# nevi-me/rust-dataframe

Hardware: AMD Instinct MI355X
Metric: rows/sec filter+sum over 1e9 f64 Arrow rows; %HBM bw at 1/2/4/8 GPU (higher is better)
Workload: dtype f64

## Files before the change

rust_dataframe_amd/csrc/rdf_capi.cpp:

```cpp
#include <hip/hip_runtime.h>

#include <algorithm>
#include <cmath>
#include <cstdarg>
#include <cstdio>
#include <chrono>
#include <functional>
#include <cstring>
#include <map>
#include <memory>
#include <mutex>
#include <condition_variable>
#include <string>
#include <thread>
#include <vector>
#include <sys/syscall.h>
#include <unistd.h>

#include "rdf_device.h"
#include "rdf_stage_copy.h"
#include "rdf_utf8.h"
#include "rdf_colstats.h"
#include "rdf_window.h"
#include "rdf_window_agg.h"
// ... 59 lines not shown
    int    opt_gb_partition = 3;
    bool   timing = false;
    std::vector<std::pair<hipEvent_t, hipEvent_t>> events;
    size_t events_used = 0;
    std::multimap<size_t, void*> pool_free;
    size_t pool_cached = 0;
    int64_t opt_stream_slab = 0;
    void*  sbuf_dev[2] = {nullptr, nullptr};
    void*  sbuf_pin[2] = {nullptr, nullptr};
    size_t sbuf_dev_cap = 0, sbuf_pin_cap = 0;
    hipEvent_t sbuf_ev[2] = {nullptr, nullptr};
    void*  dbuf_dev[2] = {nullptr, nullptr};
    void*  dbuf_pin[2] = {nullptr, nullptr};
    size_t dbuf_dev_cap = 0, dbuf_pin_cap = 0;
    hipEvent_t dbuf_ev[2] = {nullptr, nullptr};
    hipStream_t d2h_stream = nullptr;
    int64_t stream_slabs = 0, stream_bytes_staged = 0, stream_bytes_direct = 0;
    bool in_stream = false;
    bool streaming = false;
    int  opt_stream_table_kernel = 1;
    char* tab_pin = nullptr; size_t tab_pin_cap = 0, tab_pin_used = 0;
    bool   agg_comm_entered = false;
    ::rdf_comm* agg_comm = nullptr;
    ~Ctx();
};

thread_local Ctx g_ctx;

Ctx::~Ctx() {
    if (!ready || (long)syscall(SYS_gettid) == (long)getpid()) return;
    (void)hipSetDevice(device);
    if (stream) (void)hipStreamSynchronize(stream);
    for (void* p : arena.overflow) (void)hipFree(p);
    if (arena.base) (void)hipFree(arena.base);
    if (pinned) (void)hipHostFree(pinned);
    for (auto& kv : pool_free) (void)hipFree(kv.second);
    for (int b = 0; b < 2; ++b) { if (sbuf_dev[b]) (void)hipFree(sbuf_dev[b]); if (sbuf_pin[b]) (void)hipHostFree(sbuf_pin[b]); if (sbuf_ev[b]) (void)hipEventDestroy(sbuf_ev[b]); }
    if (tab_pin) (void)hipHostFree(tab_pin);
    if (d2h_stream) (void)hipStreamSynchronize(d2h_stream);
    for (int b = 0; b < 2; ++b) { if (dbuf_dev[b]) (void)hipFree(dbuf_dev[b]); if (dbuf_pin[b]) (void)hipHostFree(dbuf_pin[b]); if (dbuf_ev[b]) (void)hipEventDestroy(dbuf_ev[b]); }
    if (d2h_stream) (void)hipStreamDestroy(d2h_stream);
    for (auto& ev : events) { (void)hipEventDestroy(ev.first); (void)hipEventDestroy(ev.second); }
    if (copy_stream) { (void)hipStreamSynchronize(copy_stream); (void)hipStreamDestroy(copy_stream); }
    if (own_stream) (void)hipStreamDestroy(own_stream);
    ready = false;
}

rdf_status fail(rdf_status st, const char* fmt, ...) {
    char buf[512];
    va_list ap;
    va_start(ap, fmt);
    vsnprintf(buf, sizeof buf, fmt, ap);
    va_end(ap);
    g_ctx.err = buf;
    if (g_ctx.ready && g_ctx.stream) (void)hipStreamSynchronize(g_ctx.stream);
    return st;
}

// ... 8 lines not shown
        if (_s != RDF_OK) return _s;   \
    } while (0)

rdf_status ensure_ready() {
    Ctx& c = g_ctx;
    if (c.ready) return RDF_OK;
    int n = 0;
    hipError_t e = hipGetDeviceCount(&n);
    if (e != hipSuccess || n <= 0)
        return fail(RDF_DEVICE_ERROR, "no HIP device visible (%s); librdf_mi355x has no CPU fallback",
                    e != hipSuccess ? hipGetErrorString(e) : "device count 0");
    HIP_TRY(hipGetDevice(&c.device));
    hipDeviceProp_t prop;
    HIP_TRY(hipGetDeviceProperties(&prop, c.device));
    if (strncmp(prop.gcnArchName, "gfx950", 6) != 0)
        return fail(RDF_DEVICE_ERROR, "device %d is %s; this library carries gfx950 (MI355X) code only", c.device, prop.gcnArchName);
    HIP_TRY(hipStreamCreateWithFlags(&c.own_stream, hipStreamNonBlocking));
    c.stream = c.own_stream;
    if (const char* e = getenv("RDF_SPEC_BLOCKS_PER_CU")) { const int v = atoi(e); if (v >= 0 && v <= 8) c.opt_spec_blocks = v; }
    if (const char* e = getenv("RDF_SPEC_TILE_ROT")) c.opt_spec_tile_rot = atoi(e);
    if (const char* e = getenv("RDF_SPEC_XCD_SWZ")) c.opt_spec_xcd_swz = atoi(e);
    if (const char* e = getenv("RDF_SPEC_GRID_ADJ")) c.opt_spec_grid_adj = atoi(e);
    if (const char* e = getenv("RDF_STREAM_TABLE_KERNEL")) c.opt_stream_table_kernel = atoi(e) != 0;
    if (const char* e = getenv("RDF_GSPEC_BLOCKS_PER_CU")) { const int v = atoi(e); if (v >= 0 && v <= 8) c.opt_gspec_blocks = v; }
    c.ready = true;
    return RDF_OK;
}

void arena_begin() {
    Arena& a = g_ctx.arena;
    for (void* p : a.overflow) (void)hipFree(p);
    a.overflow.clear();
    if (a.wanted > a.cap) {
        if (a.base) (void)hipFree(a.base);
        a.base = nullptr;
        a.cap = 0;
        size_t want = a.wanted + a.wanted / 4 + (1u << 20);
        void* p = nullptr;
        if (hipMalloc(&p, want) == hipSuccess) { a.base = (char*)p; a.cap = want; }
    }
    a.used = 0;
    a.wanted = 0;
}
rdf_status arena_alloc(size_t bytes, void** out) {
    Arena& a = g_ctx.arena;
    bytes = (bytes + 16 + 255) & ~(size_t)255;
// ... 3 lines not shown
        a.used += bytes;
        return RDF_OK;
    }
    void* p = nullptr;
    hipError_t e = hipMalloc(&p, bytes);
    if (e != hipSuccess) return fail(RDF_MEMORY_ERROR, "hipMalloc(%zu) failed: %s", bytes, hipGetErrorString(e));
    a.overflow.push_back(p);
    *out = p;
    return RDF_OK;
}
rdf_status pinned_reserve(size_t bytes) {
    Ctx& c = g_ctx;
    if (bytes <= c.pinned_cap) return RDF_OK;
    if (c.pinned && c.stream) (void)hipStreamSynchronize(c.stream);
    if (c.pinned) (void)hipHostFree(c.pinned);
    c.pinned = nullptr;
    c.pinned_cap = 0;
    size_t want = bytes + bytes / 2 + 4096;
    void* p = nullptr;
    hipError_t e = hipHostMalloc(&p, want, hipHostMallocDefault);
    if (e != hipSuccess) return fail(RDF_MEMORY_ERROR, "hipHostMalloc(%zu) failed: %s", want, hipGetErrorString(e));
    c.pinned = (char*)p;
    c.pinned_cap = want;
    return RDF_OK;
}

constexpr size_t kPoolGranule = (size_t)2 << 20;
constexpr size_t kPoolMaxCached = (size_t)96 << 30;
rdf_status pool_alloc(size_t bytes, void** out, size_t* got) {
    Ctx& c = g_ctx;
    const size_t gran = bytes < ((size_t)1 << 20) ? (size_t)4096 : kPoolGranule;
    const size_t want = (bytes + 256 + gran - 1) / gran * gran;
    auto it = c.pool_free.lower_bound(want);
    if (it != c.pool_free.end() && it->first <= want + want / 4 + gran) {
        *out = it->second; *got = it->first;
        c.pool_cached -= it->first;
        c.pool_free.erase(it);
        return RDF_OK;
    }
    void* p = nullptr;
    hipError_t e = hipMalloc(&p, want);
    if (e != hipSuccess && !c.pool_free.empty()) {
        if (c.stream) (void)hipStreamSynchronize(c.stream);
        for (auto& kv : c.pool_free) (void)hipFree(kv.second);
        c.pool_free.clear();
        c.pool_cached = 0;
// ... 732 lines not shown
                    h = (sw ? mir : fwd)[op - RDF_OP_GT];
                } else if (op == RDF_OP_AND) h = LH_AND;
                else if (op == RDF_OP_OR) h = LH_OR;
                else if (in.dtype == RDF_F64) {
                    if (op == RDF_OP_ADD) h = LH_F_ADD;
                    else if (op == RDF_OP_MUL) h = LH_F_MUL;
                    else if (op == RDF_OP_SUB) h = sw ? LH_F_RSUB : LH_F_SUB;
                    else if (op == RDF_OP_DIV) h = sw ? LH_F_RDIV : LH_F_DIV;
                } else if (in.dtype == RDF_I64 || in.dtype == RDF_U64) {
                    if (op == RDF_OP_ADD) h = LH_I_ADD;
                    else if (op == RDF_OP_MUL) h = LH_I_MUL;
                    else if (op == RDF_OP_SUB) h = sw ? LH_I_RSUB : LH_I_SUB;
                }
            } break;
            default: break;
        }
        if (h == LH_NONE) return false;
        lean.code[i].swapped = (uint8_t)((in.swapped & 1) | (h << 1));
    }
    return true;
}

rdf_status launch_agg_pair(const EvalArgs* ea, const FilterAggF64Args* fa, int cmp, int feat, int grid, int nvalues,
                           const int* cls, AggPartial* partials, AggPartial* result, const char* spec_sig = nullptr,
                           const SpecArgs* sa = nullptr) {
    Ctx& c = g_ctx;
    KernelTimer kt;
    if (sa) {
        const bool jit = jit_find(spec_sig) != nullptr;
        c.last_kernel = std::string("spec_kernel<") + spec_sig + ">" + (jit ? " [compiled at run time]" : "");
        const hipError_t le = launch_spec(spec_sig, *sa, grid, c.stream);
        if (le != hipSuccess && jit) { (void)hipGetLastError(); return kRetryInterpreted; }
        if (le != hipSuccess) return fail(RDF_DEVICE_ERROR, "launch_spec: %s", hipGetErrorString(le));
    }
    else if (fa) { c.last_kernel = "filter_agg_f64_kernel"; HIP_TRY(launch_filter_agg_f64(*fa, cmp, grid, c.stream)); }
    else {
        EvalArgs lean;
        if (c.opt_interp_lean && feat == 0 && lean_assign(*ea, lean)) { c.last_kernel = "eval_kernel<AGG, lean>"; HIP_TRY(launch_eval_lean(lean, SINK_AGG, grid, c.stream, c.opt_interp_lean == 2)); }
        else { c.last_kernel = "eval_kernel<AGG>"; HIP_TRY(launch_eval(*ea, SINK_AGG, feat, grid, c.stream)); }
    }
    kt.stop();
    AggFinalArgs f;
    memset(&f, 0, sizeof f);
    f.partials = partials;
    f.result = result;
    f.nblocks = grid;
    f.nvalues = nvalues;
    for (int k = 0; k < nvalues; ++k) f.value_cls[k] = cls[k];
    HIP_TRY(launch_agg_final(f, c.stream));
    return RDF_OK;
}

void fill_agg_result(rdf_agg_result* r, int dt, const AggPartial& p) {
    memset(r, 0, sizeof *r);
    r->dtype = dt;
    r->count = p.cnt;
    r->is_some = p.cnt > 0;
    if (is_float(dt)) {
        double s, a, b;
        memcpy(&s, &p.sum, 8); memcpy(&a, &p.mn, 8); memcpy(&b, &p.mx, 8);
        r->sum_f64 = dt == RDF_F32 ? (double)(float)s : s;
        if (p.cnt > 0) { r->min_f64 = a; r->max_f64 = b; }
    } else {
        r->sum_i64 = (int64_t)h_normalize_int(dt, p.sum);
// ... 601 lines not shown
                cmp = fr.op;
                if (L.kind == RDF_NODE_COLUMN && R.kind == RDF_NODE_SCALAR) { coln = &L; sc = &R; }
                else if (L.kind == RDF_NODE_SCALAR && R.kind == RDF_NODE_COLUMN) {
                    coln = &R; sc = &L;
                    cmp = fr.op == RDF_OP_GT ? RDF_OP_LT : fr.op == RDF_OP_GE ? RDF_OP_LE : fr.op == RDF_OP_LT ? RDF_OP_GT : fr.op == RDF_OP_LE ? RDF_OP_GE : fr.op;
                }
                if (coln && col_dtype[coln->column] == RDF_F64 && sc->dtype != RDF_NULLTYPE && (is_numeric(sc->dtype) || sc->dtype == RDF_BOOL)) {
                    const DevChunkCol& x = in_dev[(size_t)coln->column];
                    const DevChunkCol& y = in_dev[(size_t)vr.column];
                    const uintptr_t xa = (uintptr_t)((const double*)x.values + x.offset), ya = (uintptr_t)((const double*)y.values + y.offset);
                    if ((xa & 7) == 0 && (ya & 7) == 0 && (xa & 15) == (ya & 15)) {
                        memset(&fa, 0, sizeof fa);
                        fa.x = (const double*)x.values; fa.x_validity = x.validity; fa.x_offset = x.offset;
                        fa.y = (const double*)y.values; fa.y_validity = y.validity; fa.y_offset = y.offset;
                        fa.n = clen[0];
                        const uint64_t cu = cc.imm_for(*sc, RDF_F64);
                        memcpy(&fa.c, &cu, 8);
                        fa.partials = d_partials;
                        fast = true;
                    }
                }
            }
        }
        if (use_spec) {
            const rdf_status ls = launch_agg_pair(nullptr, nullptr, 0, 0, grid, ps.nvalues, cls, d_partials, d_result, sp.sig.c_str(), &sa);
            if (ls == kRetryInterpreted) return run_program(ps, cols, ncols, nchunks, outs, aggs, len_mismatch_msg, fc);
            RDF_TRY(ls);
        } else if (fast) {
            const int64_t per_block = (int64_t)kBlock * 4 * 2;
            int64_t want = (clen[0] + per_block - 1) / per_block;
            grid = (int)(want < (int64_t)eval_grid_limit() ? want : (int64_t)eval_grid_limit());
            if (grid < 1) grid = 1;
            d_result = d_partials + (size_t)grid * (size_t)ps.nvalues;
            RDF_TRY(launch_agg_pair(nullptr, &fa, cmp, 0, grid, 1, cls, d_partials, d_result));
        } else {
            RDF_TRY(launch_agg_pair(&ea, nullptr, 0, cc.feat(), grid, ps.nvalues, cls, d_partials, d_result));
        }
        if (ctx.agg_comm) {
            AggPartial hp[kMaxValues];
            uint32_t flags = 0;
            RDF_TRY(agg_dist_finish(*ctx.agg_comm, d_result, d_flags, ps.nvalues, cls, hp, &flags));
            if (flags & 2u) return fail(RDF_COMPUTE_ERROR, "pipeline_dist: another rank failed before the combine");
            if (flags & 1u) return fail(RDF_DIVIDE_BY_ZERO, "Divide by zero error");
            for (int v = 0; v < ps.nvalues; ++v) fill_agg_result(&aggs[v], value_dtype[v], hp[v]);
            return RDF_OK;
        }
        RDF_TRY(pinned_reserve(pin_off + 64 + sizeof(AggPartial) * kMaxValues));
        char* pin = ctx.pinned + pin_off;
        HIP_TRY(hipMemcpyAsync(pin, d_flags, 16, hipMemcpyDeviceToHost, ctx.stream));
        HIP_TRY(hipMemcpyAsync(pin + 64, d_result, sizeof(AggPartial) * (size_t)ps.nvalues, hipMemcpyDeviceToHost, ctx.stream));
        HIP_TRY(hipStreamSynchronize(ctx.stream));
        dbg.mark("kernel + result");
        uint32_t flags;
        memcpy(&flags, pin, 4);
        if (flags & 1u) return fail(RDF_DIVIDE_BY_ZERO, "Divide by zero error");
        for (int v = 0; v < ps.nvalues; ++v) {
            AggPartial p;
            memcpy(&p, pin + 64 + sizeof(AggPartial) * (size_t)v, sizeof p);
            fill_agg_result(&aggs[v], value_dtype[v], p);
        }
        return RDF_OK;
    }

    {
        KernelTimer kt;
        if (use_spec) {
            const bool jit = jit_find(sp.sig.c_str()) != nullptr;
            ctx.last_kernel = "spec_kernel<" + sp.sig + ">" + (jit ? " [compiled at run time]" : "");
            const hipError_t le = launch_spec(sp.sig.c_str(), sa, grid, ctx.stream);
            if (le != hipSuccess && jit) { (void)hipGetLastError(); return run_program(ps, cols, ncols, nchunks, outs, aggs, len_mismatch_msg, fc); }
            if (le != hipSuccess) return fail(RDF_DEVICE_ERROR, "launch_spec: %s", hipGetErrorString(le));
        }
        else {
            int64_t longest = 0;
            for (int64_t i = 0; i < nchunks; ++i) longest = std::max(longest, clen[(size_t)i]);
            EvalArgs lean;
            if (ctx.opt_interp_lean && cc.feat() == 0 && longest < ((int64_t)1 << 32) && lean_assign(ea, lean, SINK_STORE)) {
// ... 105 lines not shown
rdf_status rdf_device_count(int32_t* count) {
    if (!count) return fail(RDF_INVALID_ARGUMENT, "null pointer");
    int n = 0;
    hipError_t e = hipGetDeviceCount(&n);
    *count = e == hipSuccess ? n : 0;
    if (e != hipSuccess) return fail(RDF_DEVICE_ERROR, "hipGetDeviceCount: %s", hipGetErrorString(e));
    return RDF_OK;
}

rdf_status rdf_set_device(int32_t device) {
    Ctx& c = g_ctx;
    if (c.ready && c.device == device) return RDF_OK;
    if (c.ready) {
        (void)hipStreamSynchronize(c.stream);
        for (void* p : c.arena.overflow) (void)hipFree(p);
        c.arena.overflow.clear();
        if (c.arena.base) (void)hipFree(c.arena.base);
        c.arena = Arena();
        for (auto& ev : c.events) { (void)hipEventDestroy(ev.first); (void)hipEventDestroy(ev.second); }
        c.events.clear();
        c.events_used = 0;
        if (c.own_stream) (void)hipStreamDestroy(c.own_stream);
        c.own_stream = c.stream = nullptr;
        c.ready = false;
    }
    HIP_TRY(hipSetDevice(device));
    return ensure_ready();
}

rdf_status rdf_set_stream(void* hip_stream) {
    RDF_TRY(ensure_ready());
    g_ctx.stream = hip_stream ? (hipStream_t)hip_stream : g_ctx.own_stream;
    return RDF_OK;
}

rdf_status rdf_synchronize(void) {
    RDF_TRY(ensure_ready());
    HIP_TRY(hipStreamSynchronize(g_ctx.stream));
    return RDF_OK;
}

rdf_status rdf_dev_alloc(void** ptr, int64_t bytes) {
    if (!ptr || bytes < 0) return fail(RDF_INVALID_ARGUMENT, "bad arguments");
    RDF_TRY(ensure_ready());
    void* p = nullptr;
    hipError_t e = hipMalloc(&p, (size_t)bytes + 64);
// ... 2089 lines not shown
    RDF_TRY(ensure_ready());
    if (n > 0) HIP_TRY(launch_fill_f64(dev_ptr, n, seed, column_id, first_row, lo, hi, g_ctx.stream));
    HIP_TRY(hipStreamSynchronize(g_ctx.stream));
    return RDF_OK;
}
rdf_status rdf_fill_uniform_i64(int64_t* dev_ptr, int64_t n, uint64_t seed, uint64_t column_id, int64_t first_row, int64_t lo, int64_t hi) {
    if (hi <= lo) return fail(RDF_INVALID_ARGUMENT, "fill_uniform_i64: hi must exceed lo");
    RDF_TRY(ensure_ready());
    if (n > 0) HIP_TRY(launch_fill_i64(dev_ptr, n, seed, column_id, first_row, lo, hi, g_ctx.stream));
    HIP_TRY(hipStreamSynchronize(g_ctx.stream));
    return RDF_OK;
}
rdf_status rdf_fill_validity(uint8_t* dev_ptr, int64_t nbits, uint64_t seed, uint64_t column_id, int64_t first_row, double null_fraction) {
    RDF_TRY(ensure_ready());
    if (nbits > 0) HIP_TRY(launch_fill_validity(dev_ptr, nbits, seed, column_id, first_row, null_fraction, g_ctx.stream));
    HIP_TRY(hipStreamSynchronize(g_ctx.stream));
    return RDF_OK;
}

rdf_status rdf_set_option(const char* name, int64_t value) {
    if (!name) return fail(RDF_INVALID_ARGUMENT, "null option name");
    if (strcmp(name, "spec") == 0) g_ctx.opt_spec = value != 0;
    else if (strcmp(name, "fast_filter") == 0) g_ctx.opt_fast_filter = value != 0;
    else if (strcmp(name, "vec_bitmap") == 0) g_ctx.opt_vec_bitmap = value != 0;
    else if (strcmp(name, "gb_partition") == 0) g_ctx.opt_gb_partition = value == 2 ? 3 : (int)value;
    else if (strcmp(name, "gb_debug") == 0) g_ctx.opt_gb_debug = value == 3 ? 3 : 0;
    else if (strcmp(name, "filter_tile") == 0) g_ctx.opt_filter_tile = (int)value;
    else if (strcmp(name, "filter_one") == 0) g_ctx.opt_filter_one = value != 0;
    else if (strcmp(name, "take_rows") == 0) g_ctx.opt_take_rows = (int)value;
    else if (strcmp(name, "sort_gen") == 0 || strcmp(name, "sort_pipe") == 0 || strcmp(name, "sort_super") == 0) {}
    else if (strcmp(name, "sort_msd") == 0) g_ctx.opt_sort_msd = (int)value;
    else if (strcmp(name, "sort_sample") == 0) g_ctx.opt_sort_sample = (int)value;
    else if (strcmp(name, "stream_table_kernel") == 0) g_ctx.opt_stream_table_kernel = value != 0;
    else if (strcmp(name, "join_table") == 0) g_ctx.opt_join_table = value < 0 || value > 2 ? 2 : (int)value;
    else if (strcmp(name, "jit") == 0) g_ctx.opt_jit = (int)value;
    else if (strcmp(name, "gb_skew_plan") == 0) g_ctx.opt_gb_skew_plan = (int)value;
    else if (strcmp(name, "gb_compact") == 0) g_ctx.opt_gb_compact = (int)value;
    else if (strcmp(name, "gb_bucket") == 0) g_ctx.opt_gb_bucket = (int)value;
    else if (strcmp(name, "gb_hot") == 0) g_ctx.opt_gb_hot = (int)value;
    else if (strcmp(name, "spec_blocks_per_cu") == 0) g_ctx.opt_spec_blocks = (int)value;
    else if (strcmp(name, "spec_tile_rot") == 0) g_ctx.opt_spec_tile_rot = value < 0 ? -1 : (int)value;
    else if (strcmp(name, "spec_xcd_swz") == 0) g_ctx.opt_spec_xcd_swz = value < 0 ? -1 : value != 0;
    else if (strcmp(name, "spec_grid_adj") == 0) g_ctx.opt_spec_grid_adj = (int)value;
    else if (strcmp(name, "gspec_blocks_per_cu") == 0) g_ctx.opt_gspec_blocks = (int)value;
    else if (strcmp(name, "filter_gen") == 0) g_ctx.opt_filter_gen = (int)value;
    else if (strcmp(name, "filter_fused") == 0) g_ctx.opt_filter_fused = (int)value;
// ... 90 lines not shown
```

rust_dataframe_amd/csrc/rdf_common.hip.h:

```cpp
#pragma once
#include "rdf_device.h"

namespace rdfk {

__device__ __forceinline__ uint64_t uniform64(uint64_t v) {
    uint32_t lo = __builtin_amdgcn_readfirstlane((uint32_t)v);
    uint32_t hi = __builtin_amdgcn_readfirstlane((uint32_t)(v >> 32));
    return ((uint64_t)hi << 32) | lo;
}
__device__ __forceinline__ int wave_id() { return __builtin_amdgcn_readfirstlane((int)(threadIdx.x >> 6)); }

template <class T> using GlobalPtr = const T __attribute__((address_space(1)))*;
template <class T> using GlobalMutPtr = T __attribute__((address_space(1)))*;
template <class T> __device__ __forceinline__ GlobalPtr<T> as_global(const void* p) { return (GlobalPtr<T>)p; }
template <class T> using ConstPtr = const T __attribute__((address_space(4)))*;
template <class T> __device__ __forceinline__ ConstPtr<T> as_const(const void* p) { return (ConstPtr<T>)p; }
__device__ __forceinline__ DevChunkCol const_col(const DevChunkCol* table, int64_t i) {
    const ConstPtr<DevChunkCol> t = as_const<DevChunkCol>(table);
    DevChunkCol c;
    c.values = t[i].values; c.validity = t[i].validity; c.offset = t[i].offset;
    return c;
}
template <class T> __device__ __forceinline__ GlobalMutPtr<T> as_global_mut(void* p) { return (GlobalMutPtr<T>)p; }

// ... 109 lines not shown
    if (cls == CLS_F64) { sum = d2u(0.0); mn = mx = 0x7FF8000000000000ull; }
    else if (cls == CLS_SIGNED) { sum = 0; mn = (uint64_t)INT64_MAX; mx = (uint64_t)INT64_MIN; }
    else { sum = 0; mn = ~0ull; mx = 0; }
}
__device__ __forceinline__ void agg_merge(int cls, uint64_t& sum, uint64_t& mn, uint64_t& mx, int64_t& cnt,
                                          uint64_t s2, uint64_t mn2, uint64_t mx2, int64_t c2) {
    cnt += c2;
    if (cls == CLS_F64) {
        sum = d2u(u2d(sum) + u2d(s2));
        mn = d2u(fmin(u2d(mn), u2d(mn2)));
        mx = d2u(fmax(u2d(mx), u2d(mx2)));
    } else if (cls == CLS_SIGNED) {
        sum += s2;
        mn = (uint64_t)((int64_t)mn2 < (int64_t)mn ? (int64_t)mn2 : (int64_t)mn);
        mx = (uint64_t)((int64_t)mx2 > (int64_t)mx ? (int64_t)mx2 : (int64_t)mx);
    } else {
        sum += s2;
        mn = mn2 < mn ? mn2 : mn;
        mx = mx2 > mx ? mx2 : mx;
    }
}

__device__ __forceinline__ void block_reduce_agg(int cls, uint64_t sum, uint64_t mn, uint64_t mx, int64_t cnt,
                                                 AggPartial* lds4, AggPartial* out) {
#pragma unroll
    for (int m = 32; m >= 1; m >>= 1) {
        uint64_t s2 = shfl_xor64(sum, m), mn2 = shfl_xor64(mn, m), mx2 = shfl_xor64(mx, m);
        int64_t c2 = (int64_t)shfl_xor64((uint64_t)cnt, m);
        agg_merge(cls, sum, mn, mx, cnt, s2, mn2, mx2, c2);
    }
    const int wave = threadIdx.x >> 6;
    __syncthreads();
    if ((threadIdx.x & 63) == 0) { lds4[wave].sum = sum; lds4[wave].mn = mn; lds4[wave].mx = mx; lds4[wave].cnt = cnt; }
    __syncthreads();
    if (threadIdx.x == 0) {
        uint64_t s = lds4[0].sum, a = lds4[0].mn, b = lds4[0].mx;
        int64_t c = lds4[0].cnt;
        for (int w = 1; w < kBlock / 64; ++w) agg_merge(cls, s, a, b, c, lds4[w].sum, lds4[w].mn, lds4[w].mx, lds4[w].cnt);
        out->sum = s; out->mn = a; out->mx = b; out->cnt = c;
    }
}

__device__ __forceinline__ void trig_reduce(double x, double& r, int& q) {
    const double kd = rint(x * 6.36619772367581382433e-01);
    q = (int)kd;
    double t = fma(-kd, 1.57079632673412561417e+00, x);
    t = fma(-kd, 6.07710050630396597660e-11, t);
    t = fma(-kd, 2.02226624871116645580e-21, t);
    r = fma(-kd, 8.47842766036889956997e-32, t);
}
__device__ __forceinline__ double trig_ksin(double r) {
    const double z = r * r, v = z * r;
    const double p = fma(z, fma(z, fma(z, fma(z, 1.58969099521155010221e-10, -2.50507602534068634195e-08), 2.75573137070700676789e-06),
                                -1.98412698298579493134e-04), 8.33333333332248946124e-03);
    return fma(v, fma(z, p, -1.66666666666666324348e-01), r);
}
__device__ __forceinline__ double trig_kcos(double r) {
    const double z = r * r;
    const double p = z * fma(z, fma(z, fma(z, fma(z, fma(z, -1.13596475577881948265e-11, 2.08757232129817482790e-09), -2.75573143513906633035e-07),
                                            2.48015872894767294178e-05), -1.38888888888741095749e-03), 4.16666666666666019037e-02);
    return 1.0 - (0.5 * z - z * p);
}
// ... 214 lines not shown
```

rust_dataframe_amd/csrc/rdf_device.h:

```cpp
#pragma once
#include "rdf_sort_map.h"
#include <stdint.h>
#include <hip/hip_runtime.h>

#include <string>
#include "../../include/rdf_mi355x.h"

namespace rdfk {

constexpr int kBlock = 256;
constexpr int kVPT = 4;
constexpr int kEvalTile = kBlock * kVPT;
constexpr int kFilterTile = 4096;
constexpr int kFilterTileSmall = 1024;
constexpr int kMaxCode = 56;
constexpr int kMaxCols = 8;
constexpr int kMaxFrameCols = 64;
constexpr int kPreCols = 4;
constexpr int kMaxTmp = 4;
constexpr int kMaxValues = RDF_MAX_VALUES;
constexpr int kMaxGroupValues = RDF_MAX_GROUP_VALUES;
constexpr int kMaxFilterCols = 8;

struct DevChunkCol {
// ... 13 lines not shown
    uint8_t  bc;
    uint8_t  op;
    uint8_t  dtype;
    uint8_t  src_kind;
    uint8_t  src_dtype;
    uint8_t  swapped;
    uint16_t src;
    uint64_t imm;
};
static_assert(sizeof(Instr) == 16, "Instr must stay 16 bytes");
enum : int {
    LH_NONE = 0, LH_LOAD, LH_STORE_TMP, LH_FILTER, LH_EMIT, LH_NOT, LH_CAST_I2F, LH_CAST_U2F,
    LH_F_GT, LH_F_GE, LH_F_EQ, LH_F_NE, LH_F_LT, LH_F_LE, LH_F_ADD, LH_F_SUB, LH_F_RSUB, LH_F_MUL, LH_F_DIV, LH_F_RDIV,
    LH_I_ADD, LH_I_SUB, LH_I_RSUB, LH_I_MUL, LH_AND, LH_OR
};

struct AggPartial {
    uint64_t sum, mn, mx;
    int64_t  cnt;
};
enum : int32_t { CLS_F64 = 0, CLS_SIGNED = 1, CLS_UNSIGNED = 2 };

enum : int32_t { SINK_STORE = 0, SINK_AGG = 1, SINK_GROUP = 2 };

struct EvalArgs {
    const DevChunkCol* cols;
    const int64_t*     chunk_tile_start;
    const int64_t*     chunk_len;
    DevOutChunk*       outs;
    int64_t*           out_null_counts;
    AggPartial*        partials;
    uint64_t*          group_partials;
    uint32_t*          flags;
    int64_t            nchunks, ntiles;
    DevChunkCol        inline_cols[kMaxCols];
    DevOutChunk        inline_outs[kMaxValues];
    int64_t            inline_len;
    int32_t            ncols, nvalues, ncode, ntmp;
    int32_t            col_dtype[kMaxCols];
    int32_t            value_cls[kMaxGroupValues];
    int32_t            ngroups, group_replicas;
    Instr              code[kMaxCode];
};

inline __host__ __device__ int group_words(int ngroups, int nvalues) { return (ngroups + 1) * (2 * nvalues + 1); }

constexpr int kGSpecCols = 8;
constexpr int kGSpecImm = 8;
struct GSpecArgs {
    const DevChunkCol* cols_tab;
    const int64_t*     chunk_tile_start;
    const int64_t*     chunk_len;
    DevChunkCol        cols[kGSpecCols];
    int32_t            col_map[kGSpecCols];
    int64_t            nchunks, ntiles, n;
    uint64_t           imm[kGSpecImm];
    uint64_t*          group_partials;
    uint32_t*          flags;
    int32_t            ngroups, nvalues, vec_bitmap;
    int32_t            xcd_swz, tile_rot, pad1;
};

struct GroupFinalArgs {
    const uint64_t* partials;
    uint64_t*       result;
    int32_t         nblocks, words, ngroups, nvalues;
    int32_t         value_cls[kMaxGroupValues];
};

struct AggFinalArgs {
    const AggPartial* partials;
    AggPartial*       result;
    int32_t           nblocks, nvalues;
    int32_t           value_cls[kMaxValues];
};

struct FilterAggF64Args {
    const double*  x;   const uint8_t* x_validity;   int64_t x_offset;
    const double*  y;   const uint8_t* y_validity;   int64_t y_offset;
    int64_t        n;
    double         c;
    AggPartial*    partials;
};

constexpr int kSpecCols = 8;
constexpr int kSpecImm = 8;
struct SpecArgs {
    DevChunkCol        cols[kSpecCols];
    DevOutChunk        out;
    const DevChunkCol* cols_tab;
    const DevOutChunk* outs_tab;
    const int64_t*     chunk_tile_start;
    const int64_t*     chunk_len;
    int64_t            nchunks, ntiles;
    int64_t            n;
    uint64_t           tile_inv;
    uint64_t           imm[kSpecImm];
    int64_t*           out_null_count;
    AggPartial*        partials;
    uint32_t*          flags;
    int32_t            vec_bitmap;
    int32_t            rt[8];
    int32_t            alias[kSpecCols];
    int64_t            tile_rot;
    int32_t            xcd_swz, pad0;
};

struct MaskTables {
    const DevChunkCol* mask;
    const int64_t*     chunk_tile_start;
    const int64_t*     chunk_len;
    int64_t            nchunks, ntiles;
};
struct FilterArgs {
    MaskTables         t;
    const DevChunkCol* cols;
    DevOutChunk*       outs;
    int64_t*           out_null_counts;
    const int64_t*     tile_scan;
    int32_t            ncols;
    int32_t            esize[kMaxFilterCols];
};

struct FilterOneArgs {
    DevChunkCol        mask;
    int64_t            clen, ntiles;
    const int64_t*     tile_scan;
    int64_t*           out_null_counts;
// ... 471 lines not shown
```

rust_dataframe_amd/csrc/rdf_eval.hip:

```cpp
#include "rdf_common.hip.h"

#ifndef RDF_FEAT
#error "compile with -DRDF_FEAT=0|1|2"
#endif

namespace rdfk {


__device__ __forceinline__ uint64_t cast_value(int from, int to, uint64_t x, bool& ok) {
    ok = true;
    if (from == to) return x;
    double f = 0.0;
    bool src_float = false;
    if (from == RDF_F64) { f = u2d(x); src_float = true; }
    else if (from == RDF_F32) { f = (double)u2f(x); src_float = true; }
    if (to == RDF_BOOL) return src_float ? (uint64_t)(f != 0.0) : (uint64_t)(x != 0);
    if (to == RDF_F64) {
        if (src_float) return d2u(f);
        return d2u(dt_is_signed(from) ? (double)(int64_t)x : (double)x);
    }
    if (to == RDF_F32) {
        if (from == RDF_F64) return f2u((float)u2d(x));
        return f2u(dt_is_signed(from) ? (float)(int64_t)x : (float)x);
    }
// ... 657 lines not shown
#pragma unroll
        for (int k = 0; k < NVAL; ++k)
            if (k < a.nvalues && nullacc[k])
                atomicAdd((unsigned long long*)&a.out_null_counts[(int64_t)k * a.nchunks + cur_chunk], (unsigned long long)nullacc[k]);
    }
    if (err) atomicOr(a.flags, err);
    if (SINK == SINK_GROUP) {
        __syncthreads();
        for (int w = tid; w < gwords; w += kBlock) {
            const bool fsum = w < a.nvalues * gS && a.value_cls[(w / gS) & (kMaxGroupValues - 1)] == CLS_F64;
            uint64_t acc0 = gtab[w];
            for (int r = 1; r < a.group_replicas; ++r) {
                const uint64_t x = gtab[(size_t)r * gwords + w];
                acc0 = fsum ? d2u(u2d(acc0) + u2d(x)) : acc0 + x;
            }
            a.group_partials[(size_t)blockIdx.x * gwords + w] = acc0;
        }
    }
    if (SINK == SINK_AGG) {
#pragma unroll
        for (int k = 0; k < NVAL; ++k)
            if (k < a.nvalues)
                block_reduce_agg(a.value_cls[k], g_sum[k], g_mn[k], g_mx[k], g_cnt[k], red_lds,
                                 &a.partials[(int64_t)blockIdx.x * a.nvalues + k]);
    }
}


template <int SINK, int NPRE, int NVAL>
static void launch_one(const EvalArgs& a, int grid, size_t lds, hipStream_t s) {
    hipLaunchKernelGGL((eval_kernel<RDF_FEAT, SINK, NPRE, NVAL>), dim3(grid), dim3(kBlock), lds, s, a);
}
template <int SINK>
static void launch_shape(const EvalArgs& a, int npre, int nval, int grid, size_t lds, hipStream_t s) {
    if (nval <= 1) {
        if (npre <= 1) launch_one<SINK, 1, 1>(a, grid, lds, s);
        else if (npre <= 2) launch_one<SINK, 2, 1>(a, grid, lds, s);
        else launch_one<SINK, 4, 1>(a, grid, lds, s);
    } else if (nval <= 2) {
        if (npre <= 2) launch_one<SINK, 2, 2>(a, grid, lds, s);
        else launch_one<SINK, 4, 2>(a, grid, lds, s);
    } else launch_one<SINK, 4, 4>(a, grid, lds, s);
}

#define RDF_CAT2(a, b) a##b
#define RDF_CAT(a, b) RDF_CAT2(a, b)
hipError_t RDF_CAT(launch_eval_feat, RDF_FEAT)(const EvalArgs& a, int sink, int grid, hipStream_t s) {
// ... 14 lines not shown
```

rust_dataframe_amd/csrc/rdf_kernels.hip:

```cpp
#include "rdf_common.hip.h"
#include "rdf_join_place.h"

namespace rdfk {

__global__ __launch_bounds__(kBlock) void agg_final_kernel(const AggFinalArgs a) {
    __shared__ AggPartial red_lds[kBlock / 64];
    for (int k = 0; k < a.nvalues; ++k) {
        const int cls = a.value_cls[k];
        uint64_t s, mn, mx;
        int64_t cnt;
        agg_init(cls, s, mn, mx, cnt);
        for (int b = threadIdx.x; b < a.nblocks; b += kBlock) {
            const AggPartial p = a.partials[(int64_t)b * a.nvalues + k];
            agg_merge(cls, s, mn, mx, cnt, p.sum, p.mn, p.mx, p.cnt);
        }
        block_reduce_agg(cls, s, mn, mx, cnt, red_lds, &a.result[k]);
        __syncthreads();
    }
}


template <int CMP>
__device__ __forceinline__ bool cmp_f64(double x, double c) {
    if (CMP == RDF_OP_GT) return x > c;
    if (CMP == RDF_OP_GE) return x >= c;
    if (CMP == RDF_OP_EQ) return x == c;
    if (CMP == RDF_OP_NE) return x != c;
    if (CMP == RDF_OP_LT) return x < c;
    return x <= c;
}

struct F64Agg {
    double sum, mn, mx;
    int64_t cnt;
    __device__ __forceinline__ void init() { sum = 0.0; mn = mx = __longlong_as_double(0x7FF8000000000000ll); cnt = 0; }
    __device__ __forceinline__ void add(double v) { sum += v; mn = fmin(mn, v); mx = fmax(mx, v); ++cnt; }
};

constexpr int kFU = 4;
typedef double dvec2 __attribute__((ext_vector_type(2)));

// ... 41 lines not shown
                if (!SAME) vy[u] = (dvec2)(0.0);
            }
        }
        uint64_t wx[2 * kFU], wy[2 * kFU];
        if (HASV) {
            const int64_t rw = 2 * wbase;
            if (a.x_validity) load_windows<2 * kFU>(a.x_validity, a.x_offset + head + rw, body_rows - rw, wx);
            if (!SAME && a.y_validity) load_windows<2 * kFU>(a.y_validity, a.y_offset + head + rw, body_rows - rw, wy);
        }
#pragma unroll
        for (int u = 0; u < kFU; ++u) {
            const int64_t i = wbase + u * 64 + lane;
            uint32_t bits = i < nvec ? 3u : 0u;
            if (HASV) {
                const int sh = (2 * lane) & 63;
                if (a.x_validity) bits &= (uint32_t)((lane < 32 ? wx[2 * u] : wx[2 * u + 1]) >> sh) & 3u;
                if (!SAME && a.y_validity) bits &= (uint32_t)((lane < 32 ? wy[2 * u] : wy[2 * u + 1]) >> sh) & 3u;
            }
            const dvec2 yy = SAME ? vx[u] : vy[u];
            if ((bits & 1u) && cmp_f64<CMP>(vx[u].x, a.c)) g.add(yy.x);
            if ((bits & 2u) && cmp_f64<CMP>(vx[u].y, a.c)) g.add(yy.y);
        }
    }
    block_reduce_agg(CLS_F64, d2u(g.sum), d2u(g.mn), d2u(g.mx), g.cnt, red_lds, &a.partials[blockIdx.x]);
}

template <int WW> constexpr int filter_tile_rows() { return WW * 64 * (kBlock / 64); }
static_assert(filter_tile_rows<16>() == kFilterTile && filter_tile_rows<4>() == kFilterTileSmall, "tile sizes of the two instantiations");

template <int WW>
__device__ __forceinline__ void locate_tile(const MaskTables& t, int64_t tile, int64_t& c, int64_t& r0, int64_t& clen) {
    c = t.nchunks == 1 ? 0 : find_chunk_tile(t.chunk_tile_start, t.nchunks, tile);
    r0 = (tile - t.chunk_tile_start[c]) * filter_tile_rows<WW>();
    clen = t.chunk_len[c];
}

template <int kWW>
__device__ __forceinline__ void keep_words(const DevChunkCol& m, int64_t rw, int64_t clen, uint64_t (&kw)[kWW]) {
    load_windows<kWW>((const uint8_t*)m.values, m.offset + rw, clen - rw, kw);
    if (m.validity) {
        uint64_t vw[kWW];
        load_windows<kWW>(m.validity, m.offset + rw, clen - rw, vw);
#pragma unroll
        for (int i = 0; i < kWW; ++i) kw[i] &= vw[i];
    }
}

// ... 1331 lines not shown
```

rust_dataframe_amd/csrc/rdf_spec_kernel.hip.h:

```cpp
#pragma once
#include <map>
#include <string>
#include <type_traits>

#include "rdf_expr.hip.h"

namespace rdfk {


template <int DT> struct AggT;
template <> struct AggT<RDF_F64> {
    double sum, mn, mx; int64_t cnt;
    static constexpr int cls = CLS_F64;
    __device__ __forceinline__ void init() { sum = 0.0; mn = mx = __longlong_as_double(0x7FF8000000000000ll); cnt = 0; }
    __device__ __forceinline__ void add(double v) { sum += v; mn = fmin(mn, v); mx = fmax(mx, v); ++cnt; }
    __device__ __forceinline__ uint64_t s() const { return d2u(sum); }
    __device__ __forceinline__ uint64_t a() const { return d2u(mn); }
    __device__ __forceinline__ uint64_t b() const { return d2u(mx); }
};
template <> struct AggT<RDF_I64> {
    uint64_t sum; int64_t mn, mx; int64_t cnt;
    static constexpr int cls = CLS_SIGNED;
    __device__ __forceinline__ void init() { sum = 0; mn = INT64_MAX; mx = INT64_MIN; cnt = 0; }
    __device__ __forceinline__ void add(int64_t v) { sum += (uint64_t)v; mn = v < mn ? v : mn; mx = v > mx ? v : mx; ++cnt; }
// ... 395 lines not shown
#pragma unroll
                        for (int e = 0; e < RV; ++e) if ((inu >> e) & 1) as_global_mut<So>(out.values)[(int64_t)RV * i + e] = (So)x[e];
                    }
                }
                if (out.validity) {
#pragma unroll
                    for (int h = 0; h < RV; ++h) {
                        const uint64_t wv = interleave_word<RV>(vb, h, lane);
                        if (lane == RV * u + h) word_vld = wv;
                    }
                }
#pragma unroll
                for (int e = 0; e < RV; ++e) nulls += (uint32_t)__popcll(inb[e] & ~vb[e]);
            }
            if (lane < R && rw + 64 * lane < n) {
                if constexpr (V0::dt == RDF_BOOL) as_global_mut<uint64_t>(out.values)[(rw >> 6) + lane] = word_val;
                if (out.validity) as_global_mut<uint64_t>(out.validity)[(rw >> 6) + lane] = word_vld;
            }
        }
    }
    if (c.err) atomicOr(a.flags, c.err);
    if constexpr (P::SINK == SINK_AGG) {
        constexpr int nv = has_v1 ? 2 : 1;
        block_reduce_agg(g0.cls, g0.s(), g0.a(), g0.b(), g0.cnt, red_lds, &a.partials[(int64_t)blockIdx.x * nv]);
        if constexpr (has_v1) block_reduce_agg(g1.cls, g1.s(), g1.a(), g1.b(), g1.cnt, red_lds, &a.partials[(int64_t)blockIdx.x * nv + 1]);
    } else {
        if (cur_chunk >= 0 && lane == 0 && nulls) atomicAdd((unsigned long long*)&a.out_null_count[cur_chunk], (unsigned long long)nulls);
    }
}


typedef void (*SpecLaunch)(const SpecArgs&, int, hipStream_t);
struct SpecEntry { SpecLaunch launch; int rows_per_tile; };
std::map<std::string, SpecEntry>& spec_registry();

template <class P>
static void launch_prog(const SpecArgs& a, int grid, hipStream_t s) {
    hipLaunchKernelGGL((spec_kernel<P>), dim3(grid), dim3(kBlock), 0, s, a);
}
template <class P>
static void reg() { spec_registry()[P::sig()] = SpecEntry{&launch_prog<P>, 64 * P::R}; }

struct Lc; struct Lk;
template <int FROM> struct Lx;
template <class X, class Y> struct Op;
template <class X> struct Tr;
template <class Sh, int S, int C, int K, int DT> struct Build;
template <int S, int C, int K, int DT> struct Build<Lc, S, C, K, DT> {
// ... 111 lines not shown
```

Baseline: 842.2 billion.

## Fold aggregate partials in the last block and write result to mapped host memory

Adds a last-block-done pattern to the aggregation kernels. Each block writes its partial with agent-scope stores and takes an atomic ticket, and the final block folds all partials and writes the result plus flags straight into a mapped pinned host slot. This removes the separate agg_final_kernel launch and the two device-to-host memcpys per query, leaving only a stream synchronize. In exchange every block pays an atomic and a fence, and the last block does a serial fold. Correctness relies on the ticket counter at d_flags+1 being zeroed beforehand, and the lean interpreter path falls back to the old scheme.

```diff
diff --git a/rust_dataframe_amd/csrc/rdf_capi.cpp b/rust_dataframe_amd/csrc/rdf_capi.cpp
--- a/rust_dataframe_amd/csrc/rdf_capi.cpp
+++ b/rust_dataframe_amd/csrc/rdf_capi.cpp
@@ -105,6 +105,9 @@
     char* tab_pin = nullptr; size_t tab_pin_cap = 0, tab_pin_used = 0;
     bool   agg_comm_entered = false;
     ::rdf_comm* agg_comm = nullptr;
+    int    opt_agg_one_launch = 1;
+    rdfk::AggSlot* agg_slot = nullptr;
+    rdfk::AggSlot* agg_slot_dev = nullptr;
     ~Ctx();
 };
 
@@ -117,6 +120,7 @@
     for (void* p : arena.overflow) (void)hipFree(p);
     if (arena.base) (void)hipFree(arena.base);
     if (pinned) (void)hipHostFree(pinned);
+    if (agg_slot) (void)hipHostFree(agg_slot);
     for (auto& kv : pool_free) (void)hipFree(kv.second);
     for (int b = 0; b < 2; ++b) { if (sbuf_dev[b]) (void)hipFree(sbuf_dev[b]); if (sbuf_pin[b]) (void)hipHostFree(sbuf_pin[b]); if (sbuf_ev[b]) (void)hipEventDestroy(sbuf_ev[b]); }
     if (tab_pin) (void)hipHostFree(tab_pin);
@@ -171,6 +175,7 @@
     if (const char* e = getenv("RDF_SPEC_XCD_SWZ")) c.opt_spec_xcd_swz = atoi(e);
     if (const char* e = getenv("RDF_SPEC_GRID_ADJ")) c.opt_spec_grid_adj = atoi(e);
     if (const char* e = getenv("RDF_STREAM_TABLE_KERNEL")) c.opt_stream_table_kernel = atoi(e) != 0;
+    if (const char* e = getenv("RDF_AGG_ONE_LAUNCH")) c.opt_agg_one_launch = atoi(e) != 0;
     if (const char* e = getenv("RDF_GSPEC_BLOCKS_PER_CU")) { const int v = atoi(e); if (v >= 0 && v <= 8) c.opt_gspec_blocks = v; }
     c.ready = true;
     return RDF_OK;
@@ -220,6 +225,20 @@
     if (e != hipSuccess) return fail(RDF_MEMORY_ERROR, "hipHostMalloc(%zu) failed: %s", want, hipGetErrorString(e));
     c.pinned = (char*)p;
     c.pinned_cap = want;
+    return RDF_OK;
+}
+
+rdf_status agg_slot_ready() {
+    Ctx& c = g_ctx;
+    if (c.agg_slot) return RDF_OK;
+    void* p = nullptr;
+    void* d = nullptr;
+    hipError_t e = hipHostMalloc(&p, sizeof(rdfk::AggSlot), hipHostMallocDefault);
+    if (e != hipSuccess) return fail(RDF_MEMORY_ERROR, "hipHostMalloc(%zu) for the aggregate result slot failed: %s", sizeof(rdfk::AggSlot), hipGetErrorString(e));
+    e = hipHostGetDevicePointer(&d, p, 0);
+    if (e != hipSuccess) { (void)hipHostFree(p); return fail(RDF_DEVICE_ERROR, "hipHostGetDevicePointer(aggregate result slot): %s", hipGetErrorString(e)); }
+    c.agg_slot = (rdfk::AggSlot*)p;
+    c.agg_slot_dev = (rdfk::AggSlot*)d;
     return RDF_OK;
 }
 
@@ -998,10 +1017,11 @@
 }
 
 rdf_status launch_agg_pair(const EvalArgs* ea, const FilterAggF64Args* fa, int cmp, int feat, int grid, int nvalues,
-                           const int* cls, AggPartial* partials, AggPartial* result, const char* spec_sig = nullptr,
+                           const int* cls, AggPartial* partials, AggPartial* result, bool* folded, const char* spec_sig = nullptr,
                            const SpecArgs* sa = nullptr) {
     Ctx& c = g_ctx;
     KernelTimer kt;
+    *folded = sa ? sa->fin.counter != nullptr : fa ? fa->fin.counter != nullptr : ea->fin.counter != nullptr;
     if (sa) {
         const bool jit = jit_find(spec_sig) != nullptr;
         c.last_kernel = std::string("spec_kernel<") + spec_sig + ">" + (jit ? " [compiled at run time]" : "");
@@ -1012,10 +1032,11 @@
     else if (fa) { c.last_kernel = "filter_agg_f64_kernel"; HIP_TRY(launch_filter_agg_f64(*fa, cmp, grid, c.stream)); }
     else {
         EvalArgs lean;
-        if (c.opt_interp_lean && feat == 0 && lean_assign(*ea, lean)) { c.last_kernel = "eval_kernel<AGG, lean>"; HIP_TRY(launch_eval_lean(lean, SINK_AGG, grid, c.stream, c.opt_interp_lean == 2)); }
+        if (c.opt_interp_lean && feat == 0 && lean_assign(*ea, lean)) { *folded = false; c.last_kernel = "eval_kernel<AGG, lean>"; HIP_TRY(launch_eval_lean(lean, SINK_AGG, grid, c.stream, c.opt_interp_lean == 2)); }
         else { c.last_kernel = "eval_kernel<AGG>"; HIP_TRY(launch_eval(*ea, SINK_AGG, feat, grid, c.stream)); }
     }
     kt.stop();
+    if (*folded) return RDF_OK;
     AggFinalArgs f;
     memset(&f, 0, sizeof f);
     f.partials = partials;
@@ -1663,8 +1684,20 @@
                 }
             }
         }
+        AggFinish fin;
+        memset(&fin, 0, sizeof fin);
+        bool folded = false;
+        if (ctx.opt_agg_one_launch) {
+            RDF_TRY(agg_slot_ready());
+            fin.counter = d_flags + 1;
+            fin.flags = d_flags;
+            fin.slot = ctx.agg_slot_dev;
+            ctx.agg_slot->flags = kAggSlotPending;
+        }
         if (use_spec) {
-            const rdf_status ls = launch_agg_pair(nullptr, nullptr, 0, 0, grid, ps.nvalues, cls, d_partials, d_result, sp.sig.c_str(), &sa);
+            fin.result = d_result;
+            sa.fin = fin;
+            const rdf_status ls = launch_agg_pair(nullptr, nullptr, 0, 0, grid, ps.nvalues, cls, d_partials, d_result, &folded, sp.sig.c_str(), &sa);
             if (ls == kRetryInterpreted) return run_program(ps, cols, ncols, nchunks, outs, aggs, len_mismatch_msg, fc);
             RDF_TRY(ls);
         } else if (fast) {
@@ -1673,9 +1706,13 @@
             grid = (int)(want < (int64_t)eval_grid_limit() ? want : (int64_t)eval_grid_limit());
             if (grid < 1) grid = 1;
             d_result = d_partials + (size_t)grid * (size_t)ps.nvalues;
-            RDF_TRY(launch_agg_pair(nullptr, &fa, cmp, 0, grid, 1, cls, d_partials, d_result));
+            fin.result = d_result;
+            fa.fin = fin;
+            RDF_TRY(launch_agg_pair(nullptr, &fa, cmp, 0, grid, 1, cls, d_partials, d_result, &folded));
         } else {
-            RDF_TRY(launch_agg_pair(&ea, nullptr, 0, cc.feat(), grid, ps.nvalues, cls, d_partials, d_result));
+            fin.result = d_result;
+            ea.fin = fin;
+            RDF_TRY(launch_agg_pair(&ea, nullptr, 0, cc.feat(), grid, ps.nvalues, cls, d_partials, d_result, &folded));
         }
         if (ctx.agg_comm) {
             AggPartial hp[kMaxValues];
@@ -1686,14 +1723,23 @@
             for (int v = 0; v < ps.nvalues; ++v) fill_agg_result(&aggs[v], value_dtype[v], hp[v]);
             return RDF_OK;
         }
-        RDF_TRY(pinned_reserve(pin_off + 64 + sizeof(AggPartial) * kMaxValues));
-        char* pin = ctx.pinned + pin_off;
-        HIP_TRY(hipMemcpyAsync(pin, d_flags, 16, hipMemcpyDeviceToHost, ctx.stream));
-        HIP_TRY(hipMemcpyAsync(pin + 64, d_result, sizeof(AggPartial) * (size_t)ps.nvalues, hipMemcpyDeviceToHost, ctx.stream));
-        HIP_TRY(hipStreamSynchronize(ctx.stream));
+        const char* pin = nullptr;
+        if (folded) {
+            static_assert(offsetof(AggSlot, result) == 64, "result slot: 64 bytes of flags, then the values");
+            HIP_TRY(hipStreamSynchronize(ctx.stream));
+            pin = (const char*)ctx.agg_slot;
+        } else {
+            RDF_TRY(pinned_reserve(pin_off + 64 + sizeof(AggPartial) * kMaxValues));
+            char* stage = ctx.pinned + pin_off;
+            HIP_TRY(hipMemcpyAsync(stage, d_flags, 16, hipMemcpyDeviceToHost, ctx.stream));
+            HIP_TRY(hipMemcpyAsync(stage + 64, d_result, sizeof(AggPartial) * (size_t)ps.nvalues, hipMemcpyDeviceToHost, ctx.stream));
+            HIP_TRY(hipStreamSynchronize(ctx.stream));
+            pin = stage;
+        }
         dbg.mark("kernel + result");
         uint32_t flags;
         memcpy(&flags, pin, 4);
+        if (folded && flags == kAggSlotPending) return fail(RDF_DEVICE_ERROR, "%s finished without delivering its result", ctx.last_kernel.c_str());
         if (flags & 1u) return fail(RDF_DIVIDE_BY_ZERO, "Divide by zero error");
         for (int v = 0; v < ps.nvalues; ++v) {
             AggPartial p;
@@ -1845,6 +1891,8 @@
         c.events_used = 0;
         if (c.own_stream) (void)hipStreamDestroy(c.own_stream);
         c.own_stream = c.stream = nullptr;
+        if (c.agg_slot) (void)hipHostFree(c.agg_slot);
+        c.agg_slot = c.agg_slot_dev = nullptr;
         c.ready = false;
     }
     HIP_TRY(hipSetDevice(device));
@@ -3980,6 +4028,7 @@
     if (!name) return fail(RDF_INVALID_ARGUMENT, "null option name");
     if (strcmp(name, "spec") == 0) g_ctx.opt_spec = value != 0;
     else if (strcmp(name, "fast_filter") == 0) g_ctx.opt_fast_filter = value != 0;
+    else if (strcmp(name, "agg_one_launch") == 0) g_ctx.opt_agg_one_launch = value != 0;
     else if (strcmp(name, "vec_bitmap") == 0) g_ctx.opt_vec_bitmap = value != 0;
     else if (strcmp(name, "gb_partition") == 0) g_ctx.opt_gb_partition = value == 2 ? 3 : (int)value;
     else if (strcmp(name, "gb_debug") == 0) g_ctx.opt_gb_debug = value == 3 ? 3 : 0;
diff --git a/rust_dataframe_amd/csrc/rdf_common.hip.h b/rust_dataframe_amd/csrc/rdf_common.hip.h
--- a/rust_dataframe_amd/csrc/rdf_common.hip.h
+++ b/rust_dataframe_amd/csrc/rdf_common.hip.h
@@ -155,7 +155,7 @@
 }
 
 __device__ __forceinline__ void block_reduce_agg(int cls, uint64_t sum, uint64_t mn, uint64_t mx, int64_t cnt,
-                                                 AggPartial* lds4, AggPartial* out) {
+                                                 AggPartial* lds4, AggPartial* out, AggPartial* out2 = nullptr, bool through = false) {
 #pragma unroll
     for (int m = 32; m >= 1; m >>= 1) {
         uint64_t s2 = shfl_xor64(sum, m), mn2 = shfl_xor64(mn, m), mx2 = shfl_xor64(mx, m);
@@ -170,7 +170,55 @@
         uint64_t s = lds4[0].sum, a = lds4[0].mn, b = lds4[0].mx;
         int64_t c = lds4[0].cnt;
         for (int w = 1; w < kBlock / 64; ++w) agg_merge(cls, s, a, b, c, lds4[w].sum, lds4[w].mn, lds4[w].mx, lds4[w].cnt);
-        out->sum = s; out->mn = a; out->mx = b; out->cnt = c;
+        if (through) {
+            __hip_atomic_store(&out->sum, s, __ATOMIC_RELAXED, __HIP_MEMORY_SCOPE_AGENT);
+            __hip_atomic_store(&out->mn, a, __ATOMIC_RELAXED, __HIP_MEMORY_SCOPE_AGENT);
+            __hip_atomic_store(&out->mx, b, __ATOMIC_RELAXED, __HIP_MEMORY_SCOPE_AGENT);
+            __hip_atomic_store(&out->cnt, c, __ATOMIC_RELAXED, __HIP_MEMORY_SCOPE_AGENT);
+        } else { out->sum = s; out->mn = a; out->mx = b; out->cnt = c; }
+        if (out2) { out2->sum = s; out2->mn = a; out2->mx = b; out2->cnt = c; }
+    }
+}
+
+template <class ClsOf>
+__device__ __forceinline__ void agg_fold_partials(const AggPartial* partials, int nblocks, int nvalues, ClsOf cls_of,
+                                                  AggPartial* lds4, AggPartial* result, AggPartial* result2 = nullptr) {
+    for (int k = 0; k < nvalues; ++k) {
+        const int cls = cls_of(k);
+        uint64_t s, mn, mx;
+        int64_t cnt;
+        agg_init(cls, s, mn, mx, cnt);
+        for (int b = threadIdx.x; b < nblocks; b += kBlock) {
+            const AggPartial p = partials[(int64_t)b * nvalues + k];
+            agg_merge(cls, s, mn, mx, cnt, p.sum, p.mn, p.mx, p.cnt);
+        }
+        block_reduce_agg(cls, s, mn, mx, cnt, lds4, &result[k], result2 ? &result2[k] : nullptr);
+        __syncthreads();
+    }
+}
+
+__device__ __forceinline__ bool agg_through(const AggFinish& f) { return f.counter != nullptr; }
+template <class ClsOf>
+__device__ __forceinline__ void agg_finish(const AggFinish& f, AggPartial* partials, int nvalues, ClsOf cls_of, AggPartial* lds4) {
+    if (f.counter == nullptr) return;
+    asm volatile("s_waitcnt vmcnt(0)" ::: "memory");
+    __syncthreads();
+    if (threadIdx.x == 0) {
+        const uint32_t ticket = __hip_atomic_fetch_add(f.counter, 1u, __ATOMIC_RELAXED, __HIP_MEMORY_SCOPE_AGENT);
+        lds4[0].cnt = ticket == gridDim.x - 1 ? 1 : 0;
+    }
+    __syncthreads();
+    const int last = __builtin_amdgcn_readfirstlane((int)lds4[0].cnt);
+    if (!last) return;
+    if (threadIdx.x == 0) {
+        __builtin_amdgcn_fence(__ATOMIC_ACQUIRE, "agent");
+        asm volatile("s_waitcnt vmcnt(0)" ::: "memory");
+    }
+    __syncthreads();
+    agg_fold_partials(partials, (int)gridDim.x, nvalues, cls_of, lds4, f.result, f.slot->result);
+    if (threadIdx.x == 0) {
+        f.slot->flags = __hip_atomic_load(f.flags, __ATOMIC_RELAXED, __HIP_MEMORY_SCOPE_AGENT);
+        __threadfence_system();
     }
 }
 
diff --git a/rust_dataframe_amd/csrc/rdf_device.h b/rust_dataframe_amd/csrc/rdf_device.h
--- a/rust_dataframe_amd/csrc/rdf_device.h
+++ b/rust_dataframe_amd/csrc/rdf_device.h
@@ -59,6 +59,19 @@
 enum : int32_t { CLS_F64 = 0, CLS_SIGNED = 1, CLS_UNSIGNED = 2 };
 
 enum : int32_t { SINK_STORE = 0, SINK_AGG = 1, SINK_GROUP = 2 };
+
+struct AggSlot {
+    uint32_t   flags;
+    uint32_t   pad[15];
+    AggPartial result[kMaxValues];
+};
+constexpr uint32_t kAggSlotPending = 0xFFFFFFFFu;
+struct AggFinish {
+    uint32_t*   counter;
+    uint32_t*   flags;
+    AggPartial* result;
+    AggSlot*    slot;
+};
 
 struct EvalArgs {
     const DevChunkCol* cols;
@@ -77,6 +90,7 @@
     int32_t            col_dtype[kMaxCols];
     int32_t            value_cls[kMaxGroupValues];
     int32_t            ngroups, group_replicas;
+    AggFinish          fin;
     Instr              code[kMaxCode];
 };
 
@@ -118,6 +132,7 @@
     int64_t        n;
     double         c;
     AggPartial*    partials;
+    AggFinish      fin;
 };
 
 constexpr int kSpecCols = 8;
@@ -141,6 +156,7 @@
     int32_t            alias[kSpecCols];
     int64_t            tile_rot;
     int32_t            xcd_swz, pad0;
+    AggFinish          fin;
 };
 
 struct MaskTables {
diff --git a/rust_dataframe_amd/csrc/rdf_eval.hip b/rust_dataframe_amd/csrc/rdf_eval.hip
--- a/rust_dataframe_amd/csrc/rdf_eval.hip
+++ b/rust_dataframe_amd/csrc/rdf_eval.hip
@@ -703,7 +703,8 @@
         for (int k = 0; k < NVAL; ++k)
             if (k < a.nvalues)
                 block_reduce_agg(a.value_cls[k], g_sum[k], g_mn[k], g_mx[k], g_cnt[k], red_lds,
-                                 &a.partials[(int64_t)blockIdx.x * a.nvalues + k]);
+                                 &a.partials[(int64_t)blockIdx.x * a.nvalues + k], nullptr, agg_through(a.fin));
+        agg_finish(a.fin, a.partials, a.nvalues, [&](int k) { return a.value_cls[k]; }, red_lds);
     }
 }
 
diff --git a/rust_dataframe_amd/csrc/rdf_kernels.hip b/rust_dataframe_amd/csrc/rdf_kernels.hip
--- a/rust_dataframe_amd/csrc/rdf_kernels.hip
+++ b/rust_dataframe_amd/csrc/rdf_kernels.hip
@@ -5,18 +5,7 @@
 
 __global__ __launch_bounds__(kBlock) void agg_final_kernel(const AggFinalArgs a) {
     __shared__ AggPartial red_lds[kBlock / 64];
-    for (int k = 0; k < a.nvalues; ++k) {
-        const int cls = a.value_cls[k];
-        uint64_t s, mn, mx;
-        int64_t cnt;
-        agg_init(cls, s, mn, mx, cnt);
-        for (int b = threadIdx.x; b < a.nblocks; b += kBlock) {
-            const AggPartial p = a.partials[(int64_t)b * a.nvalues + k];
-            agg_merge(cls, s, mn, mx, cnt, p.sum, p.mn, p.mx, p.cnt);
-        }
-        block_reduce_agg(cls, s, mn, mx, cnt, red_lds, &a.result[k]);
-        __syncthreads();
-    }
+    agg_fold_partials(a.partials, a.nblocks, a.nvalues, [&](int k) { return a.value_cls[k]; }, red_lds, a.result);
 }
 
 
@@ -104,7 +93,8 @@
             if ((bits & 2u) && cmp_f64<CMP>(vx[u].y, a.c)) g.add(yy.y);
         }
     }
-    block_reduce_agg(CLS_F64, d2u(g.sum), d2u(g.mn), d2u(g.mx), g.cnt, red_lds, &a.partials[blockIdx.x]);
+    block_reduce_agg(CLS_F64, d2u(g.sum), d2u(g.mn), d2u(g.mx), g.cnt, red_lds, &a.partials[blockIdx.x], nullptr, agg_through(a.fin));
+    agg_finish(a.fin, a.partials, 1, [](int) { return (int)CLS_F64; }, red_lds);
 }
 
 template <int WW> constexpr int filter_tile_rows() { return WW * 64 * (kBlock / 64); }
diff --git a/rust_dataframe_amd/csrc/rdf_spec_kernel.hip.h b/rust_dataframe_amd/csrc/rdf_spec_kernel.hip.h
--- a/rust_dataframe_amd/csrc/rdf_spec_kernel.hip.h
+++ b/rust_dataframe_amd/csrc/rdf_spec_kernel.hip.h
@@ -441,8 +441,9 @@
     if (c.err) atomicOr(a.flags, c.err);
     if constexpr (P::SINK == SINK_AGG) {
         constexpr int nv = has_v1 ? 2 : 1;
-        block_reduce_agg(g0.cls, g0.s(), g0.a(), g0.b(), g0.cnt, red_lds, &a.partials[(int64_t)blockIdx.x * nv]);
-        if constexpr (has_v1) block_reduce_agg(g1.cls, g1.s(), g1.a(), g1.b(), g1.cnt, red_lds, &a.partials[(int64_t)blockIdx.x * nv + 1]);
+        block_reduce_agg(g0.cls, g0.s(), g0.a(), g0.b(), g0.cnt, red_lds, &a.partials[(int64_t)blockIdx.x * nv], nullptr, agg_through(a.fin));
+        if constexpr (has_v1) block_reduce_agg(g1.cls, g1.s(), g1.a(), g1.b(), g1.cnt, red_lds, &a.partials[(int64_t)blockIdx.x * nv + 1], nullptr, agg_through(a.fin));
+        agg_finish(a.fin, a.partials, nv, [](int k) { return (int)(k == 0 ? AggT<V0::dt>::cls : AggT<V1e::dt>::cls); }, red_lds);
     } else {
         if (cur_chunk >= 0 && lane == 0 && nulls) atomicAdd((unsigned long long*)&a.out_null_count[cur_chunk], (unsigned long long)nulls);
     }
```

After: 841.7 billion (median of 3 runs). Within noise of the previous version (-0.1%).
